# simzero/cudaParticlesFoam

Hardware: AMD Instinct MI355X
Metric: Mparticle-steps/s (higher is better)
Workload: dtype f64

## Files before the change

### cudaparticlesfoam_amd/csrc/cpf_api.cpp

```cpp
#include <hip/hip_runtime.h>

#include <algorithm>
#include <cmath>
#include <cstring>
#include <limits>
#include <condition_variable>
#include <mutex>
#include <string>
#include <thread>
#include <utility>
#include <vector>

#include "cpf.h"
#include "cpf_device.h"
#include "cpf_internal.h"
#include "cpf_own.h"
#include "cpf_philox.h"
#include "cpf_walk.h"

#ifndef CPF_TIMING_EVENT_FLAGS
#define CPF_TIMING_EVENT_FLAGS hipEventReleaseToDevice
#endif

namespace {
// ... 1069 lines not shown
    CPF_REQUIRE(ctx, value != 1 && value != 2 && value != 5, CPF_ERR_ARG,
                "step_variant 1, 2 and 5 are experiments (measured slower on every mesh) and not in this build: make EXPERIMENTS=1");
#endif
    ctx->stepVariant = (int)value;
    return CPF_OK;
}

struct Option {
    const char* key;
    double lo, hi, step;
    const char* message;
    int (*set)(cpf_context*, double);
};
#define CPF_OPT(lvalue, expr) [](cpf_context* c, double v) -> int { c->lvalue = (expr); return CPF_OK; }
constexpr double kTiny = std::numeric_limits<double>::denorm_min(), kHuge = std::numeric_limits<double>::max();
const Option kOptions[] = {
    {"step_variant", -1, 5, 1, "step_variant must be -1..5", setStepVariant},
    {"vertex_fast", 0, 1, 1, "vertex_fast must be 0 or 1", CPF_OPT(vertexFast, v != 0)},
    {"z_fold", 0, 1, 1, "z_fold must be 0 or 1", CPF_OPT(zFold, v != 0)},
    {"mixed_records", 0, 1, 1, "mixed_records must be 0 or 1", CPF_OPT(mixedRecords, v != 0)},
    {"flat_walk", 0, 1, 1, "flat_walk must be 0 or 1", CPF_OPT(streamState.flat, (int)v)},
    {"flat_z", 0, 1, 1, "flat_z must be 0 or 1", CPF_OPT(streamState.flatZ, (int)v)},
    {"box_records", 0, 1, 1, "box_records must be 0 or 1", CPF_OPT(boxRecords, v != 0)},
    {"stream_tiles_per_chunk", 1, 1024, 1, "stream_tiles_per_chunk must be 1..1024", CPF_OPT(streamState.tilesPerChunk, (int)v)},
    {"sort_key_bits", 0, 0, 0, nullptr, setSortKeyBits},
    {"stream_tail_fraction", 0, 1, 0, "stream_tail_fraction must be in [0, 1]", CPF_OPT(streamState.tailFraction, v)},
    {"coop_max_cells", 0, 1 << 24, 0, "coop_max_cells must be in [0, 2^24]", CPF_OPT(streamState.coopMaxCells, (int)v)},
    {"stream_lookup", cpf::kLookupLoop - 1, cpf::kLookupBox, 1, "stream_lookup must be -1 (auto) or 0 ... 6", CPF_OPT(streamState.lookup, (int)v)},
    {"stream_lookup_by_density", 0, 1, 1, "stream_lookup_by_density must be 0 or 1", CPF_OPT(streamState.densityLookup, (int)v)},
    {"sort_method", 0, 2, 2, "sort_method must be 2 (this library's radix sort) or 0 (hipcub's)", CPF_OPT(sortMethod, (int)v)},
    {"sort_curve", -1, 1, 1, "sort_curve must be -1 (by regime), 0 (cell id) or 1 (Morton rank)", CPF_OPT(sortCurve, (int)v)},
    {"vtu_binary", 0, 1, 1, "vtu_binary must be 0 or 1", CPF_OPT(vtuBinary, v != 0)},
    {"stream_debug", 0, 0, 0, nullptr, CPF_OPT(streamState.debug, (int)v)},
    {"stream_waves_per_cu", 0, 32, 1, "stream_waves_per_cu must be 0..32 (0 = auto)", CPF_OPT(streamState.wavesPerCU, (int)v)},
    {"sort_interval", 0, 1e9, 0, "sort_interval must be >= 0 (0 = never)", CPF_OPT(sortInterval, (int)v)},
    {"timing_stride", 1, 1e6, 1, "timing_stride must be an integer >= 1", CPF_OPT(timing.stride, (int)v)},
    {"stats", 0, 0, 0, nullptr, CPF_OPT(stats, v != 0)},
    {"nonplanar_tol", kTiny, kHuge, 0, "nonplanar_tol must be a positive number", CPF_OPT(nonplanarTol, v)},
    {"split_nonplanar", 0, 1, 1, "split_nonplanar must be 0 or 1", CPF_OPT(splitNonplanar, v != 0)},
};
#undef CPF_OPT
}
extern "C" {

int cpf_set_option(cpf_context* ctx, const char* key, double value) {
    CPF_REQUIRE(ctx, ctx && key, CPF_ERR_ARG, "null argument");
    for (const Option& o : kOptions) {
        if (std::strcmp(key, o.key) != 0) continue;
        CPF_REQUIRE(ctx, !o.message || (value >= o.lo && value <= o.hi && (o.step == 0 || std::fmod(value - o.lo, o.step) == 0)),
                    CPF_ERR_ARG, o.message);
        return o.set(ctx, value);
    }
    return fail(ctx, CPF_ERR_ARG, std::string("cpf_set_option: unknown key '") + key + "'");
}

}
namespace cpf {
void set_context_error(cpf_context* ctx, const char* message) {
    if (ctx) ctx->err = message ? message : "";
}
}
extern "C" {

int cpf_step_kernel_name(cpf_context* ctx, double D, unsigned flags, char* buf, size_t bufBytes) {
    CPF_REQUIRE(ctx, ctx && buf && bufBytes > 0, CPF_ERR_ARG, "null argument");
    CPF_REQUIRE(ctx, ctx->mesh.have, CPF_ERR_STATE, "cpf_step_kernel_name: call cpf_set_mesh first");
// ... 664 lines not shown
```

### cudaparticlesfoam_amd/csrc/cpf_device.h

```cpp
#pragma once
#include <hip/hip_runtime.h>

#include <cstdint>
#include <type_traits>
#include <utility>

#include "cpf.h"
#include "cpf_internal.h"

namespace cpf {

constexpr int kBlock = 256;
constexpr int kCounterSlots = 1024;

struct MeshView {
    const int32_t* cellOff;
    const double4* planes;
    const int32_t* nbr;
    const int32_t* groupOff;
    const int32_t* groupNbr;
    const double4* U;
    const double4* cellRec;
    const double4* boxRec;
    int32_t nCells;
    int32_t allHex;
    int32_t zPairLast;
    int32_t zSide0;
    int32_t zThin;
    int32_t mixed;
};

struct GridView {
    double origin[3], invBin[3], lo[3], hi[3];
    int32_t dims[3];
    const int32_t* binOff;
    const int32_t* binCells;
};

constexpr size_t kStreamGrabBytes = 2 * 256 * 16 * sizeof(unsigned);
constexpr int kStreamHitSpillDoubles = 3 * 64;
struct StreamState {
    unsigned* d_grab = nullptr;
    double* d_hitSpill = nullptr;
    int hitSpillWaves = 0;
    int parity = 0;
    int numCU = 256;
    int tilesPerChunk = 0;
    int wavesPerCU = 0;
    int coopMaxCells = 0;
    int lookup = -1;
    double tailFraction = -1.0;
    int debug = 0;
    const volatile unsigned long long* occupiedHost = nullptr;
    int densityLookup = 0;
    bool flatField = false;
    int flat = 1;
    int flatZ = 1;
    unsigned* zBad = nullptr;
};

constexpr int kCoopMaxCells = 1 << 24;
constexpr int kFusedCoopCycles = 1 << 30;
struct VertexField;

enum : int { kLookupLoop = 0, kLookupFixed = 1, kLookupMixedBig = 2, kLookupMixed = 3, kLookupSparse = 4, kLookupMixedLoop = 5,
             kLookupBox = 6, kLookupFlatLoop = 8, kLookupFlatFixed = 9, kLookupBoxGroups = 11 };
struct LookupMode {
    int id;
    bool fixed;
    bool mixed;
    bool bigCells;
    bool box;
    bool flat;
    int gatherAhead;
};
constexpr LookupMode kLookupModes[] = {
    {kLookupLoop,       false, false, false, false, false, 0},
    {kLookupFixed,      true,  false, false, false, false, 0},
    {kLookupMixedBig,   true,  true,  true,  false, false, 0},
    {kLookupMixed,      true,  true,  false, false, false, 0},
    {kLookupSparse,     true,  false, false, false, false, 3},
    {kLookupMixedLoop,  false, true,  false, false, false, 0},
    {kLookupBox,        true,  false, false, true,  false, 0},
    {kLookupFlatLoop,   false, false, false, false, true,  0},
    {kLookupFlatFixed,  true,  false, false, false, true,  0},
// ... 143 lines not shown
```

### cudaparticlesfoam_amd/csrc/cpf_stream.hip

```cpp
#include "cpf_stream_ops.h"

#include <hip/hip_ext.h>

#include <type_traits>

namespace cpf {

#ifndef CPF_STREAM_SLOTS
#define CPF_STREAM_SLOTS 6
#endif
#ifndef CPF_STREAM_SLOTS_FIXED
#define CPF_STREAM_SLOTS_FIXED 9
#endif
#ifndef CPF_STREAM_WAVES
#define CPF_STREAM_WAVES 7
#endif
constexpr int kSlotStride = 8;
#ifndef CPF_STREAM_GATHER_LANES
#define CPF_STREAM_GATHER_LANES 32
#endif
constexpr int kStreamGatherLanes = CPF_STREAM_GATHER_LANES;
#ifndef CPF_STREAM_PAIRED
#define CPF_STREAM_PAIRED 0
#endif
// ... 62 lines not shown
#endif
#ifndef CPF_STREAM_WAVES_L2
#define CPF_STREAM_WAVES_L2 6
#endif
#ifndef CPF_STREAM_WAVES_B0
#define CPF_STREAM_WAVES_B0 7
#endif
#ifndef CPF_STREAM_HIT_POOL_B0
#define CPF_STREAM_HIT_POOL_B0 18
#endif
#ifndef CPF_STREAM_WAVES_FLAT
#define CPF_STREAM_WAVES_FLAT CPF_STREAM_WAVES
#endif
#ifndef CPF_STREAM_WAVES_FLAT_BODY
#define CPF_STREAM_WAVES_FLAT_BODY 0
#endif
#ifndef CPF_FLAT_ROUND_GATHER
#define CPF_FLAT_ROUND_GATHER 1
#endif
#ifndef CPF_FLAT_ROUND_HINTS
#define CPF_FLAT_ROUND_HINTS 1
#endif
#ifndef CPF_FLAT_ROUND_ONE_HOOK
#define CPF_FLAT_ROUND_ONE_HOOK 1
#endif
#ifndef CPF_FLAT_ROUND_MASK
#define CPF_FLAT_ROUND_MASK 1
#endif
#ifndef CPF_FLAT_ROUND_OUTCOME
#define CPF_FLAT_ROUND_OUTCOME 1
#endif
#ifndef CPF_FLAT_FACE_ASM
#define CPF_FLAT_FACE_ASM 1
#endif
#ifndef CPF_STREAM_SLOTS_BROWN
#define CPF_STREAM_SLOTS_BROWN 10
#endif
#ifndef CPF_STREAM_HIT_REGS_L2
#define CPF_STREAM_HIT_REGS_L2 0
#endif
#ifndef CPF_STREAM_WAVES_VERTEX
#define CPF_STREAM_WAVES_VERTEX 4
#endif
template <bool BROWNIAN, bool STORE_VEL, bool STATS, int LOOKUP>
struct StreamShape {
    static constexpr LookupMode mode = lookup_traits(LOOKUP);
    static_assert(mode.id == LOOKUP, "LOOKUP: a mode of kLookupModes");
    static constexpr int slots = [] {
        if (!mode.fixed) return CPF_STREAM_SLOTS;
        if (mode.box) return BROWNIAN ? CPF_STREAM_SLOTS_BOX_B : CPF_STREAM_SLOTS_BOX;
        if (BROWNIAN && LOOKUP == kLookupFixed) return CPF_STREAM_SLOTS_BROWN;
        return CPF_STREAM_SLOTS_FIXED;
    }();
    static_assert(slots >= 4 && slots <= 32, "slots");
    static constexpr int stride = mode.box ? 4 : kSlotStride;
    static constexpr bool hitInRegs = !BROWNIAN && (!mode.bigCells || CPF_STREAM_HIT_REGS_L2);
    static constexpr int pool = [] {
        if (hitInRegs) return 1;
        if (mode.mixed) return 16;
        if (BROWNIAN && LOOKUP == kLookupLoop) return CPF_STREAM_HIT_POOL_B0;
        return CPF_STREAM_HIT_POOL;
    }();
    static constexpr int waves = [] {
        if (STORE_VEL || STATS) return 1;
        if (mode.gatherAhead != 0) return BROWNIAN ? 4 : 5;
        if (BROWNIAN && mode.mixed) return 5;
// ... 19 lines not shown
              shape_is<9>(9, 7, 1, 9, 7, 40) && shape_is<11>(9, 6, 1, 12, 5, 16), "StreamShape: slots, waves, pool per mode");
#endif

template <bool BROWNIAN, bool REFLECT, bool STORE_VEL, bool STATS, int LOOKUP, bool VERTEX, bool ZSET = false>
__device__ __forceinline__ void stream_body(
    const int64_t* __restrict__ gid, double* __restrict__ vel, int64_t n, double dt, double sigma, uint32_t step0,
    int nCyc, uint32_t seed, const MeshView& m, unsigned long long* __restrict__ counters, const StreamArgs& sa, const VertexField& vf) {
    using Shape = StreamShape<BROWNIAN, STORE_VEL, STATS, LOOKUP>;
    constexpr bool LOOKUP_FIXED = Shape::mode.fixed, mixed = Shape::mode.mixed, bigCells = Shape::mode.bigCells, BOX = Shape::mode.box;
    constexpr bool FLAT = Shape::mode.flat, HIT_IN_REGS = Shape::hitInRegs;
    constexpr int kGatherAhead = Shape::mode.gatherAhead, NS = Shape::slots, kStride = Shape::stride, kPool = Shape::pool;
    constexpr unsigned kRecBytes = 32u * kStride;
    constexpr unsigned ALL = NS == 32 ? 0xFFFFFFFFu : ((1u << NS) - 1u);
    __shared__ double4 slots[NS][kStride];
    __shared__ unsigned sCnt[4];
    constexpr bool kInRound = CPF_STREAM_INROUND == 2 || (CPF_STREAM_INROUND == 1 && BROWNIAN);
    static_assert(!(kInRound && mixed), "in-round reflection knows neither face groups nor two-record cells");
    static_assert(!ZSET || (FLAT && !BROWNIAN && !VERTEX), "settled z: the flat walk without the kick or the vertex advect");
    __shared__ double sLane[ZSET ? 2 : 3][64];
    __shared__ double sPool[3][kPool];
    __shared__ unsigned sPoolUsed;
    __shared__ double sPre[ZSET ? 160 : (BROWNIAN ? 288 : 224)];
    __shared__ double sCone[VERTEX ? kVertexBlocks : 1][VERTEX ? kVertexTets * 10 : 1];
    double(*sE)[64] = sLane;
    const int lane = threadIdx.x;
    const unsigned ul = threadIdx.x;
    const unsigned preBase = uniform32(lds_addr(sPre));
    const unsigned slotBase = uniform32(lds_addr(slots));
    const int tpc = sa.tilesPerChunk;
    constexpr bool kMaskBusy = ZSET && CPF_FLAT_ROUND_MASK != 0, kPlainOutcome = ZSET && CPF_FLAT_ROUND_OUTCOME != 0;
    constexpr bool kFlatGather = ZSET && CPF_FLAT_ROUND_GATHER != 0, kHints = ZSET && CPF_FLAT_ROUND_HINTS != 0;
    constexpr bool kOneHook = ZSET && CPF_FLAT_ROUND_ONE_HOOK != 0;
    constexpr bool kFaceAsm = ZSET && CPF_FLAT_FACE_ASM != 0 && CPF_STREAM_FLAT_ZERO_SKIP == 0;
    const bool zKeep = ZSET || (FLAT && CPF_STREAM_FLAT_Z != 0 && sa.zSettled != 0);
    auto park = [&](const D3& e) __attribute__((always_inline)) {
        sE[0][lane] = e.x; sE[1][lane] = e.y;
        if (!ZSET) sE[2][lane] = e.z;
    };
    auto parked = [&]() __attribute__((always_inline)) -> D3 {
        if (ZSET) return {sE[0][lane], sE[1][lane], 0.0};
        return {sE[0][lane], sE[1][lane], sE[2][lane]};
    };
    const bool zFold = !BOX && BROWNIAN && REFLECT && m.zThin != 0;
    const bool zLast = !FLAT && !BROWNIAN && m.zPairLast != 0;
    const bool flatKick = zFold && m.zSide0 != 0;
    const unsigned nTiles = (unsigned)((n + 63) >> 6);
    const unsigned nFull = (unsigned)(n >> 6), nTail = (unsigned)n & 63u;
    const unsigned big = sa.bigChunks;
    const unsigned nChunks = big + (nTiles - big * (unsigned)tpc);
    auto chunk_first = [&](unsigned c) -> unsigned {
        return c < big ? c * (unsigned)tpc : big * (unsigned)tpc + (c - big);
    };
    auto chunk_tiles = [&](unsigned c, unsigned firstTile) -> int {
        if (c >= nChunks) return 0;
        const unsigned k = nTiles - firstTile;
        const unsigned want = c < big ? (unsigned)tpc : 1u;
        return (int)(k < want ? k : want);
    };
    auto chunk_of = [&](unsigned j) -> unsigned {
        const unsigned long long c = (unsigned long long)(blockIdx.x & (kStreamGroups - 1)) + (unsigned long long)kStreamGroups * j;
        return c < (unsigned long long)nChunks ? (unsigned)c : nChunks;
    };
    StepStats st = {0, 0, 0, 0};
#ifdef CPF_STREAM_TIMELINE
    const uint64_t tl0 = __builtin_amdgcn_s_memrealtime();
    unsigned tlTiles = 0, tlRounds = 0;
    unsigned tlWaitRec = 0, tlWaitEnd = 0, tlMissRounds = 0;
    unsigned long long* const tlH = (!STORE_VEL && vel != nullptr && (sa.debug & 4)) ? reinterpret_cast<unsigned long long*>(vel) + 8 * 16384 : nullptr;
    unsigned tlVis = 0, tlRoundIdx = 0;
#endif

    for (unsigned k = blockIdx.x; k < (unsigned)kStreamGroups; k += gridDim.x)
        if (lane == 0) sa.grabNext[k * kStreamCounterStride] = 0u;
    const unsigned grp = blockIdx.x & (kStreamGroups - 1);
    unsigned* const myGrab = sa.grab + grp * kStreamCounterStride;

    auto prefetch = [&](unsigned t, const CloudPtrs& cp) __attribute__((always_inline)) -> int {
        double* const x = cp.x; double* const y = cp.y; double* const z = cp.z; int32_t* const cell = cp.cell;
        t = uniform32(t);
        const int64_t b = (int64_t)t * 64;
        unsigned ul = threadIdx.x;
        asm volatile("" : "+v"(ul));
        if (t < nFull) {
            const char* s1 = (ul < 32u ? reinterpret_cast<const char*>(x + b) : reinterpret_cast<const char*>(y + b)) + (ul & 31u) * 16u;
            glds16(s1, preBase);
            if (zKeep) {
                if (ul < 16u) glds16(reinterpret_cast<const char*>(cell + b) + ul * 16u, preBase + 1024u);
            } else if (ul < 48u) {
                const char* s2 = ul < 32u ? reinterpret_cast<const char*>(z + b) + ul * 16u
                                          : reinterpret_cast<const char*>(cell + b) + (ul - 32u) * 16u;
                glds16(s2, preBase + 1024u);
            }
            if (BROWNIAN) {
                const int64_t* const g = CPF_STREAM_BROWN_KERNARG ? static_cast<const int64_t*>(kernarg_pointer<kKernArgGid>()) : gid;
                if (g != nullptr) {
                    if (ul < 32u) glds16(reinterpret_cast<const char*>(g + b) + ul * 16u, preBase + 1792u);
                    return 3;
                }
            }
            return 2;
        }
        const unsigned lim = nTail - 1u;
        const unsigned l = ul < lim ? ul : lim;
        if (zKeep) {
            const double vx = (x + b)[l], vy = (y + b)[l];
            const int vc = (cell + b)[l];
            sPre[ul] = vx; sPre[64 + ul] = vy;
            reinterpret_cast<int*>(sPre + 128)[ul] = vc;
        } else {
        const double vx = (x + b)[l], vy = (y + b)[l], vz = (z + b)[l];
        const int vc = (cell + b)[l];
        sPre[ul] = vx; sPre[64 + ul] = vy; sPre[128 + ul] = vz;
        reinterpret_cast<int*>(sPre + 192)[ul] = vc;
        }
        if (BROWNIAN) {
            const int64_t* const g = CPF_STREAM_BROWN_KERNARG ? static_cast<const int64_t*>(kernarg_pointer<kKernArgGid>()) : gid;
            if (g != nullptr) reinterpret_cast<int64_t*>(sPre + 224)[ul] = (g + b)[l];
        }
        return 0;
    };
// ... 29 lines not shown
                const bool haveIds = (CPF_STREAM_BROWN_KERNARG ? kernarg_pointer<kKernArgGid>() : (void*)gid) != nullptr;
                pid = haveIds ? (uint64_t) reinterpret_cast<const int64_t*>(sPre + 224)[ul] : (uint64_t)tile * 64 + ul;
            }
            if (ul > plim || pc < 0) pc = CPF_CELL_FROZEN;
            if (FLAT && !ZSET && !zKeep && ballot64(pc >= 0 && !(fabs(pz) <= 1.7976931348623157e308)) != 0ull) {
                unsigned* const bad = static_cast<unsigned*>(kernarg_pointer<kKernArgZBad>());
                if (bad != nullptr && lane == 0) *bad = 1u;
            }

            int cur = pc;
            int key2 = 0, carNext = 0, carBest = -1;
            double carDT = 2.0;
            D3 S_ = {px, py, pz}, v = {0, 0, 0};
            const uint64_t id = pid;

            unsigned ntile = 0;
            int ntilesLeft = 0;

            auto hook = [&](const D3& prev) __attribute__((always_inline)) -> int {
                int younger = 0;
                __builtin_amdgcn_sched_barrier(0);
                if (tilesLeft > 1) {
                    ntile = tile + 1;
                    ntilesLeft = tilesLeft - 1;
                } else {
                    unsigned got = 0;
                    if (lane == 0) got = grab_sync(myGrab);
                    const unsigned nxt = chunk_of(uniform32(got));
                    ntile = chunk_first(nxt);
                    ntilesLeft = chunk_tiles(nxt, ntile);
                }
                const CloudPtrs cp = kernarg_cloud_ptrs();
                double* const x = cp.x; double* const y = cp.y; double* const z = cp.z; int32_t* const cell = cp.cell;
                if (havePrev && !(sa.debug & 1)) {
                    const int64_t b = (int64_t)uniform32(rtile) * 64;
                    if (STORE_VEL && ralive) {
                        double* vv = vel + 3 * b;
                        async_store(vv, ul * 24u, rvx); async_store(vv + 1, ul * 24u, rvy); async_store(vv + 2, ul * 24u, rvz);
                    }
                    if (ul <= rlim) {
                        async_store(x + b, ul * 8u, prev.x); async_store(y + b, ul * 8u, prev.y);
                        if (!zKeep) async_store(z + b, ul * 8u, prev.z);
                        async_store(cell + b, ul * 4u, rc);
                    }
                    younger += zKeep ? 3 : 4;
                }
                if (ntilesLeft > 0 && !(sa.debug & 2)) younger += prefetch(ntile, cp);
                __builtin_amdgcn_sched_barrier(0);
                return younger;
            };

            bool busy = false;
            unsigned long long busyM = 0ull;
            bool zUnclear = false;
            int token = INT32_MIN, h = 0, j = 0;
            int hitAt = -1;
            D3 hitReg = {0, 0, 0};
            auto park_hit = [&](const D3& Hp) __attribute__((always_inline)) {
                if (HIT_IN_REGS) { hitReg = Hp; return; }
                if (hitAt < 0) hitAt = (int)atomicAdd(&sPoolUsed, 1u);
                if (hitAt < kPool) { sPool[0][hitAt] = Hp.x; sPool[1][hitAt] = Hp.y; sPool[2][hitAt] = Hp.z; }
                else {
                    double* sp = static_cast<double*>(kernarg_pointer<kKernArgHitSpill>()) + (size_t)blockIdx.x * kStreamHitSpillDoubles;
                    async_store(sp, ul * 8u, Hp.x); async_store(sp + 64, ul * 8u, Hp.y); async_store(sp + 128, ul * 8u, Hp.z);
                }
            };
// ... 109 lines not shown
                        }
#endif
                    }
                } else {
                    unsigned long long todo = busyMask;
                    missLanes = 0ull;
                    while (todo != 0ull) {
                        const int leader = __ffsll((long long)todo) - 1;
                        const int ck = __builtin_amdgcn_readlane(lk, leader);
                        const bool mine = lk == ck;
                        const unsigned long long same = ballot64(mine) & busyMask;
                        const unsigned long long hitTag = __builtin_amdgcn_uicmp((unsigned)tagv, (unsigned)ck, 32 );
                        if (hitTag != 0ull) {
                            const int sl = __ffsll((long long)hitTag) - 1;
                            used |= 1u << sl;
                            if (mine) myslot = sl;
                        } else {
                            missLanes |= same;
                        }
                        todo &= ~same;
                    }
                }
                int nJobs = 0;
                if (missLanes != 0ull) {
#define CPF_JOB(J)                                                                                          \
                    if (missLanes != 0ull && used != ALL) {                                                 \
                        const int leader = __ffsll((long long)missLanes) - 1;                               \
                        const int ck = __builtin_amdgcn_readlane(lk, leader);                               \
                        const unsigned cand = ~used & ALL;                                                  \
                        const unsigned hi = cand & (ALL << fifo) & ALL;                                     \
                        const int victim = __ffs((int)(hi ? hi : cand)) - 1;                                \
                        fifo = (unsigned)(victim + 1) == (unsigned)NS ? 0u : (unsigned)(victim + 1);          \
                        used |= 1u << victim;                                                               \
                        if (lane == victim) tagv = ck;                                                      \
                        const bool mine = lk == ck;                                                         \
                        if (mine) myslot = victim;                                                          \
                        missLanes &= ~ballot64(mine);                                                       \
                        if (ul < kRecBytes / 16u)                                                            \
                            glds16(reinterpret_cast<const char*>(BOX ? m.boxRec : m.cellRec) + (int64_t)ck * kRecBytes + ul * 16u,  \
                                   uniform32(slotBase + (unsigned)victim * kRecBytes));                     \
                        nJobs = J + 1;                                                                      \
                    }
                    CPF_JOB(0) CPF_JOB(1) CPF_JOB(2) CPF_JOB(3)
                    if (LOOKUP_FIXED) { CPF_JOB(4) CPF_JOB(5) CPF_JOB(6) CPF_JOB(7) }
#undef CPF_JOB
                }
                int younger = 0;
                if (hookDue) younger = hook(Epre);
                if (BROWNIAN && cycleStart && busy) {
                    uint32_t kStep0 = step0, kSeed = seed;
                    if (CPF_STREAM_BROWN_KERNARG) kernarg_u32_pair<kKernArgStep0, kKernArgSeed>(kStep0, kSeed);
                    const D3 xi = normal3(id, kStep0 + (uint32_t)c, kSeed);
                    sE[0][lane] = xi.x; sE[1][lane] = xi.y; sE[2][lane] = xi.z;
                }
#ifdef CPF_STREAM_TIMELINE
                const uint64_t tlw0 = __builtin_amdgcn_s_memrealtime();
#endif
                if (nJobs != 0) {
                    if (ZSET) {
                        if (younger == 5) wait_vmcnt<5>();
                        else if (younger == 3) wait_vmcnt<3>();
                        else if (younger == 2) wait_vmcnt<2>();
                        else wait_vmcnt<0>();
                    } else
                    if (younger >= 7) wait_vmcnt<7>();
                    else if (younger == 6) wait_vmcnt<6>();
                    else if (younger == 5) wait_vmcnt<5>();
                    else if (younger >= 4) wait_vmcnt<4>();
                    else if (younger == 3) wait_vmcnt<3>();
                    else if (younger >= 2) wait_vmcnt<2>();
                    else wait_vmcnt<0>();
#ifdef CPF_STREAM_TIMELINE
                    tlWaitRec += (unsigned)(__builtin_amdgcn_s_memrealtime() - tlw0); ++tlMissRounds;
#endif
                }
                const bool gatherRound = __popcll(missLanes) >= kStreamGatherLanes;
                auto advect = [&](const double4* rec) __attribute__((always_inline)) -> D3 {
                    D3 Pn;
                    if (VERTEX) {
                        Pn = {S_.x + dt * v.x, S_.y + dt * v.y, S_.z + dt * v.z};
                    } else {
                        double4 u;
                        if (BOX) { const double2 uxy = reinterpret_cast<const double2*>(rec)[5]; u = {uxy.x, uxy.y, reinterpret_cast<const double*>(rec)[12], 0.0}; }
                        else u = rec[6];
                        v = {u.x, u.y, u.z};
                        if (ZSET) Pn = {fma(dt, v.x, S_.x), fma(dt, v.y, S_.y), 0.0};
                        else Pn = axpy(dt, v, S_);
                    }
                    D3 disp = {Pn.x - S_.x, Pn.y - S_.y, ZSET ? 0.0 : Pn.z - S_.z};
                    if (BROWNIAN) {
                        const D3 xi = {sE[0][lane], sE[1][lane], sE[2][lane]};
// ... 204 lines not shown
                    }
#endif
                    if (live > 0) cycle_end();
#ifdef CPF_STREAM_CAP_TEST
                    if (capDropped) { S_ = capKeep; cur = capCur; }
#endif
                }
            } else {
                const D3 prev = parked();
                (void)hook(prev);
            }

#ifdef CPF_STREAM_TIMELINE
            const uint64_t tle0 = __builtin_amdgcn_s_memrealtime();
#endif
            wait_vmcnt<0>();
#ifdef CPF_STREAM_TIMELINE
            tlWaitEnd += (unsigned)(__builtin_amdgcn_s_memrealtime() - tle0);
            ++tlTiles;
#endif
            rtile = tile; havePrev = true;
            park(S_);
            if (STORE_VEL) { rvx = v.x; rvy = v.y; rvz = v.z; ralive = pc >= 0; }
            rc = cur;
            rlim = plim;
            if (ntilesLeft <= 0) break;
            tile = ntile; tilesLeft = ntilesLeft;
        }
        {
            const int64_t b = (int64_t)rtile * 64;
            const CloudPtrs cp = kernarg_cloud_ptrs();
            double* const x = cp.x; double* const y = cp.y; double* const z = cp.z; int32_t* const cell = cp.cell;
            const D3 res = parked();
            if (ul <= rlim) {
                (x + b)[ul] = res.x; (y + b)[ul] = res.y;
                if (!zKeep) (z + b)[ul] = res.z;
                (cell + b)[ul] = rc;
            }
            if (STORE_VEL && ralive) {
                double* vv = vel + 3 * b;
                vv[3 * ul] = rvx; vv[3 * ul + 1] = rvy; vv[3 * ul + 2] = rvz;
            }
        }
    }
#ifdef CPF_STREAM_TIMELINE
    if (!STORE_VEL && vel != nullptr && lane == 0) {
        uint64_t* o = reinterpret_cast<uint64_t*>(vel) + 8 * (uint64_t)blockIdx.x;
        o[0] = tl0; o[1] = __builtin_amdgcn_s_memrealtime(); o[2] = tlTiles; o[3] = tlRounds;
        o[4] = tlWaitRec; o[5] = tlWaitEnd; o[6] = tlMissRounds; o[7] = 0;
    }
#endif
    if (STATS) flush_stats(st, counters, sCnt);
}

template <bool BROWNIAN, bool REFLECT, bool STORE_VEL, bool STATS, int LOOKUP>
__global__ __launch_bounds__(64, (StreamShape<BROWNIAN, STORE_VEL, STATS, LOOKUP>::waves)) void step_kernel_stream(
    double* __restrict__ , double* __restrict__ , double* __restrict__ , int32_t* __restrict__ ,
    const int64_t* __restrict__ gid, double* __restrict__ vel, int64_t n, double dt, double sigma, uint32_t step0,
    int nCyc, uint32_t seed, MeshView m, unsigned long long* __restrict__ counters, StreamArgs sa) {
    stream_body<BROWNIAN, REFLECT, STORE_VEL, STATS, LOOKUP, false>(gid, vel, n, dt, sigma, step0, nCyc, seed, m, counters, sa, VertexField{});
}

template <bool BROWNIAN, bool REFLECT, bool STORE_VEL, bool STATS, int LOOKUP>
__global__ __launch_bounds__(64, ((STORE_VEL || STATS) ? 1 : CPF_STREAM_WAVES_VERTEX)) void step_kernel_stream_vertex(
    double* __restrict__ , double* __restrict__ , double* __restrict__ , int32_t* __restrict__ ,
    const int64_t* __restrict__ gid, double* __restrict__ vel, int64_t n, double dt, double sigma, uint32_t step0,
    int nCyc, uint32_t seed, MeshView m, unsigned long long* __restrict__ counters, StreamArgs sa, VertexField vf) {
    stream_body<BROWNIAN, REFLECT, STORE_VEL, STATS, LOOKUP, true>(gid, vel, n, dt, sigma, step0, nCyc, seed, m, counters, sa, vf);
}

template <bool REFLECT, bool STORE_VEL, bool STATS, int LOOKUP>
__global__ __launch_bounds__(64, (StreamShape<false, STORE_VEL, STATS, LOOKUP>::waves)) void step_kernel_stream_flat(
    double* __restrict__ , double* __restrict__ , double* __restrict__ , int32_t* __restrict__ ,
    const int64_t* __restrict__ gid, double* __restrict__ vel, int64_t n, double dt, double sigma, uint32_t step0,
// ... 22 lines not shown
        else if constexpr (ZS) return &step_kernel_stream_flat<R_, SV, ST, LF>;
        else return &step_kernel_stream<B, R_, SV, ST, LF>;
    }();
    static int wavesPerCU = 0;
    if (wavesPerCU == 0) {
        int nb = 0;
        const hipError_t e = hipOccupancyMaxActiveBlocksPerMultiprocessor(&nb, kernel, 64, 0);
        if (e != hipSuccess) return e;
        wavesPerCU = nb < 1 ? 1 : (nb > 32 ? 32 : nb);
        if (ZS && CPF_STREAM_WAVES_FLAT_BODY > 0 && wavesPerCU > 4 * CPF_STREAM_WAVES_FLAT_BODY) wavesPerCU = 4 * CPF_STREAM_WAVES_FLAT_BODY;
    }
    const int64_t nTiles = (n + 63) >> 6;
    if (nTiles >= ((int64_t)1 << 31)) return hipErrorInvalidValue;
    const int64_t slotsOnChip = (int64_t)((ss.wavesPerCU > 0 && !VX) ? ss.wavesPerCU : wavesPerCU) * ss.numCU;
    int tpc = ss.tilesPerChunk > 0 ? ss.tilesPerChunk : (!mode.fixed ? 4 : 3);
    const double tailFraction = ss.tailFraction >= 0.0 ? ss.tailFraction : (!mode.fixed ? 0.1 : 0.2);
    while (tpc > 1 && nTiles / tpc < 4 * slotsOnChip) tpc = tpc > 2 ? tpc - 1 : 1;
    int64_t bigChunks = (int64_t)((double)(nTiles / tpc) * (1.0 - tailFraction));
    if (tpc == 1 || bigChunks < 0) bigChunks = 0;
    const int64_t nChunks = bigChunks + (nTiles - bigChunks * tpc);
    int64_t R = slotsOnChip / kStreamGroups;
    const int64_t need = (nChunks + kStreamGroups - 1) / kStreamGroups;
    if (R > need) R = need;
    if (R < 1) R = 1;
    unsigned* cur = ss.d_grab + (size_t)(ss.parity & 1) * kStreamGroups * kStreamCounterStride;
    unsigned* nxt = ss.d_grab + (size_t)((ss.parity & 1) ^ 1) * kStreamGroups * kStreamCounterStride;
    if (R * kStreamGroups > ss.hitSpillWaves) R = ss.hitSpillWaves / kStreamGroups;
    if (R < 1 || ss.d_hitSpill == nullptr) return hipErrorInvalidValue;
    const bool zSettled = mode.flat && !VX && settled && ss.flatZ != 0;
    if (ZS != zSettled && mode.flat && !VX) return hipErrorInvalidValue;
    StreamArgs sa = {cur, nxt, (int)R, tpc, (unsigned)bigChunks, ss.debug, ss.d_hitSpill, zSettled ? 1 : 0, ss.zBad};
    auto launch = [&](const auto&... tail) {
        const dim3 grid((unsigned)(R * kStreamGroups));
        if (evStart != nullptr && evStop != nullptr)
            hipExtLaunchKernelGGL(kernel, grid, dim3(64), 0, st, evStart, evStop, 0, x, y, z, cell, gid, vel, n, dt, sigma, step0, nCyc,
                                  seed, m, counters, sa, tail...);
        else
            hipLaunchKernelGGL(kernel, grid, dim3(64), 0, st, x, y, z, cell, gid, vel, n, dt, sigma, step0, nCyc, seed, m, counters, sa,
                               tail...);
        return stream_launch_done(st, ss);
    };
    if constexpr (VX) return vf == nullptr ? hipErrorInvalidValue : launch(*vf);
    else return launch();
}

static int stream_lookup_mode(int64_t n, const MeshView& m, const StreamState& ss, bool brown, bool vertex) {
    int64_t cells = m.nCells;
    if (ss.densityLookup && ss.occupiedHost != nullptr) {
        const int64_t occ = (int64_t)ss.occupiedHost[0], live = (int64_t)ss.occupiedHost[1];
        if (occ > 0 && occ <= cells && live > 0 && live <= 2 * n && n <= 2 * live) cells = occ;
    }
    if (vertex) {
        if (ss.lookup == kLookupLoop || ss.lookup == kLookupFixed) return ss.lookup;
        return n < 128 * cells ? kLookupFixed : kLookupLoop;
    }
    if (m.mixed == 1 && m.boxRec != nullptr && m.zThin == 0 && ss.lookup < 0) return kLookupBoxGroups;
    if (m.mixed == 2) return kLookupMixedBig;
    if (m.mixed) return (ss.lookup >= 0 ? ss.lookup == kLookupLoop : n >= 128 * cells) ? kLookupMixedLoop : kLookupMixed;
    const bool box = m.boxRec != nullptr && m.zThin == 0;
    if (ss.lookup >= 0) return (ss.lookup == kLookupBox && !box) ? kLookupFixed : ss.lookup;
    if (box && CPF_STREAM_BOX_SPARSE) return kLookupBox;
    if (n < kStreamSparsePerCell * cells) return kLookupSparse;
    const bool flat = !brown && ss.flat && ss.flatField && m.zSide0 != 0;
    if (n < 128 * cells) return flat ? kLookupFlatFixed : kLookupFixed;
    return flat ? kLookupFlatLoop : kLookupLoop;
}

StepPlan plan_step(const MeshView& m, const StreamState& ss, int variant, const VertexField* vf, int64_t n, int nCyc, double D,
                   unsigned flags, bool stats) {
    StepPlan p;
    p.brown = D > 0.0;
    p.reflect = (flags & CPF_STEP_NO_REFLECT) == 0;
    p.storeVel = (flags & CPF_STEP_STORE_VEL) != 0;
    p.stats = stats;
    const int coopMaxCells = (ss.coopMaxCells <= 0 || ss.coopMaxCells > kCoopMaxCells) ? kCoopMaxCells : ss.coopMaxCells;
    if (!m.allHex) {
// ... 11 lines not shown
    if (vf != nullptr) {
        p.cone = vf->cone != nullptr;
        const bool streams = p.cone && vf->tetsPerCell == 12 && m.mixed == 0 && m.cellRec != nullptr && variant == kVariantStream;
        p.kernel = streams ? StepPlan::kStreamVertex : StepPlan::kVertex;
        if (streams) p.lookup = stream_lookup_mode(n, m, ss, p.brown, true);
        return p;
    }
    if (variant == kVariantAhead && (p.brown || p.storeVel || nCyc != 1)) variant = kVariantStream;
    p.kernel = (StepPlan::Kernel)variant;
    if (variant == kVariantStream) p.lookup = stream_lookup_mode(n, m, ss, p.brown, false);
    return p;
}

constexpr bool vertex_mode(LookupMode r) { return !(r.mixed || r.box || r.flat || r.gatherAhead != 0); }
hipError_t launch_step_stream(const StepPlan& p, hipStream_t st, double* x, double* y, double* z, int32_t* cell, const int64_t* gid,
                              double* vel, int64_t n, double dt, double sigma, uint32_t step0, int nCyc, uint32_t seed,
                              const MeshView& m, unsigned long long* counters, const VertexField* vf, StreamState& ss, bool zSettled,
                              hipEvent_t evStart, hipEvent_t evStop) {
    return with_bools([&](auto B, auto R, auto SV, auto ST) {
        auto inst = [&](auto kick, auto LF, auto VX, auto ZS) {
            return launch_stream_inst<kick, R, SV, ST, LF, VX, ZS>(st, x, y, z, cell, gid, vel, n, dt, sigma, step0, nCyc, seed, m, counters,
                                                                   ss, vf, zSettled, evStart, evStop);
        };
        constexpr std::true_type yes{}; constexpr std::false_type no{};
        if (p.kernel == StepPlan::kStreamVertex)
            return with_lookup(p.lookup, [&](auto LF) {
                if constexpr (vertex_mode(lookup_traits(LF))) return inst(B, LF, yes, no);
                else return hipErrorInvalidValue;
            });
        const bool body = p.flat_body(ss, zSettled);
        return with_lookup(p.lookup, [&](auto LF) {
            if constexpr (!lookup_traits(LF).flat) return inst(B, LF, no, no);
            else if constexpr (B) return hipErrorInvalidValue;
            else return body ? inst(no, LF, no, yes) : inst(no, LF, no, no);
        });
    }, p.brown, p.reflect, p.storeVel, p.stats);
}

}
```

### cudaparticlesfoam_amd/csrc/cpf_stream_ops.h

```cpp
#pragma once
#include "cpf_walk.h"

namespace cpf {

#ifndef CPF_STREAM_GROUPS
#define CPF_STREAM_GROUPS 256
#endif
constexpr int kStreamGroups = CPF_STREAM_GROUPS;
constexpr int kStreamCounterStride = 16;

typedef __attribute__((address_space(3))) const char* lds_cptr;
__device__ __forceinline__ unsigned lds_addr(const void* p) {
    return (unsigned)(uintptr_t)(lds_cptr)p;
}
__device__ __forceinline__ unsigned uniform32(unsigned v) { return (unsigned)__builtin_amdgcn_readfirstlane((int)v); }
__device__ __forceinline__ int64_t uniform64(int64_t v) {
    const unsigned lo = uniform32((unsigned)v), hi = uniform32((unsigned)((uint64_t)v >> 32));
    return (int64_t)(((uint64_t)hi << 32) | lo);
}
__device__ __forceinline__ void glds16(const void* gsrc, unsigned ldsDst) {
    unsigned keep;
    asm volatile("s_waitcnt lgkmcnt(0)\n\ts_mov_b32 %0, m0\n\ts_mov_b32 m0, %2\n\ts_nop 0\n\t"
                 "global_load_lds_dwordx4 %1, off\n\ts_mov_b32 m0, %0"
                 : "=&s"(keep) : "v"(gsrc), "s"(ldsDst) : "memory");
}
__device__ __forceinline__ void async_store(double* base, unsigned byteOff, double v) {
    asm volatile("s_nop 4\n\tglobal_store_dwordx2 %0, %1, %2" : : "v"(byteOff), "v"(v), "s"(base) : "memory");
}
__device__ __forceinline__ void async_store(int32_t* base, unsigned byteOff, int v) {
    asm volatile("s_nop 4\n\tglobal_store_dword %0, %1, %2" : : "v"(byteOff), "v"(v), "s"(base) : "memory");
}
__device__ __forceinline__ unsigned grab_sync(unsigned* base) {
    unsigned r;
    asm volatile("s_nop 4\n\tglobal_atomic_add %0, %1, %2, %3 sc0\n\ts_waitcnt vmcnt(0)" : "=&v"(r) : "v"(0u), "v"(1u), "s"(base) : "memory");
    return r;
}
__device__ __forceinline__ void load3_sync(const double* base, unsigned byteOff, double& a, double& b, double& c) {
    asm volatile("s_waitcnt vmcnt(0)\n\ts_nop 4\n\tglobal_load_dwordx2 %0, %3, %4 sc0 sc1\n\tglobal_load_dwordx2 %1, %3, %4 offset:512 sc0 sc1\n\t"
                 "global_load_dwordx2 %2, %3, %4 offset:1024 sc0 sc1\n\ts_waitcnt vmcnt(0)"
                 : "=&v"(a), "=&v"(b), "=&v"(c) : "v"(byteOff), "s"(base) : "memory");
}
struct CloudPtrs { double* x; double* y; double* z; int32_t* cell; };
__device__ __forceinline__ CloudPtrs kernarg_cloud_ptrs() {
    typedef unsigned u32x8 __attribute__((ext_vector_type(8)));
    u32x8 r;
    asm volatile("s_load_dwordx8 %0, %1, 0x0\n\ts_waitcnt lgkmcnt(0)" : "=s"(r) : "s"(__builtin_amdgcn_kernarg_segment_ptr()) : "memory");
    auto ptr = [](unsigned lo, unsigned hi) { return (uintptr_t)(((unsigned long long)hi << 32) | lo); };
    return {reinterpret_cast<double*>(ptr(r[0], r[1])), reinterpret_cast<double*>(ptr(r[2], r[3])),
            reinterpret_cast<double*>(ptr(r[4], r[5])), reinterpret_cast<int32_t*>(ptr(r[6], r[7]))};
}
template <int BYTE_OFFSET>
__device__ __forceinline__ void* kernarg_pointer() {
    typedef unsigned u32x2 __attribute__((ext_vector_type(2)));
    u32x2 r;
    asm volatile("s_load_dwordx2 %0, %1, %2\n\ts_waitcnt lgkmcnt(0)" : "=s"(r) : "s"(__builtin_amdgcn_kernarg_segment_ptr()), "n"(BYTE_OFFSET) : "memory");
    return reinterpret_cast<void*>((uintptr_t)(((unsigned long long)r[1] << 32) | r[0]));
}
template <int OFF_A, int OFF_B>
__device__ __forceinline__ void kernarg_u32_pair(uint32_t& a, uint32_t& b) {
    asm volatile("s_load_dword %0, %2, %3\n\ts_load_dword %1, %2, %4\n\ts_waitcnt lgkmcnt(0)"
                 : "=&s"(a), "=&s"(b) : "s"(__builtin_amdgcn_kernarg_segment_ptr()), "n"(OFF_A), "n"(OFF_B) : "memory");
}
template <int BYTE_OFFSET>
__device__ __forceinline__ double kernarg_f64() {
    typedef unsigned u32x2 __attribute__((ext_vector_type(2)));
    u32x2 r;
    asm volatile("s_load_dwordx2 %0, %1, %2\n\ts_waitcnt lgkmcnt(0)" : "=s"(r) : "s"(__builtin_amdgcn_kernarg_segment_ptr()), "n"(BYTE_OFFSET) : "memory");
    return __longlong_as_double((long long)(((unsigned long long)r[1] << 32) | r[0]));
}
template <int N>
__device__ __forceinline__ void wait_vmcnt() { asm volatile("s_waitcnt vmcnt(%0)" : : "n"(N) : "memory"); }

struct StreamArgs {
    unsigned* grab;
    unsigned* grabNext;
    int wavesPerGroup;
    int tilesPerChunk;
    unsigned bigChunks;
    int debug;
    double* hitSpill;
    int zSettled;
    unsigned* zBad;
};

inline hipError_t stream_launch_done(hipStream_t st, StreamState& ss) {
    const hipError_t e = hipGetLastError();
    if (e == hipSuccess) { ss.parity ^= 1; return e; }
    (void)hipMemsetAsync(ss.d_grab, 0, kStreamGrabBytes, st);
    return e;
}

}
```

Measured before the change: 112,400.

## Use 32-bit offsets in flat settled-z stream walk, segmenting large clouds

Adds a 32-bit offset path for the flat settled-z stream kernel. Tile loads, stores and record gathers compute unsigned byte offsets instead of 64-bit pointer arithmetic, and stores are fused into inline-asm groups. The m0-based global_load_lds variant and a branchy scalar vmcnt wait are meant to trim scalar and address instructions in the hot loop. To keep offsets within 32 bits, clouds larger than a segment size (new option) are launched in several kernels, which adds launches and splits the event timing across first and last launches.

After: 112,900 (median of 6 runs). Within noise of the previous version (+0.5%).

```diff
diff --git a/cudaparticlesfoam_amd/csrc/cpf_api.cpp b/cudaparticlesfoam_amd/csrc/cpf_api.cpp
--- a/cudaparticlesfoam_amd/csrc/cpf_api.cpp
+++ b/cudaparticlesfoam_amd/csrc/cpf_api.cpp
@@ -1125,6 +1125,8 @@
     {"sort_curve", -1, 1, 1, "sort_curve must be -1 (by regime), 0 (cell id) or 1 (Morton rank)", CPF_OPT(sortCurve, (int)v)},
     {"vtu_binary", 0, 1, 1, "vtu_binary must be 0 or 1", CPF_OPT(vtuBinary, v != 0)},
     {"stream_debug", 0, 0, 0, nullptr, CPF_OPT(streamState.debug, (int)v)},
+    {"stream_segment_particles", 64, (double)((int64_t)1 << 29), 0, "stream_segment_particles must be in [64, 2^29]",
+     CPF_OPT(streamState.segment, (int64_t)v / 64 * 64)},
     {"stream_waves_per_cu", 0, 32, 1, "stream_waves_per_cu must be 0..32 (0 = auto)", CPF_OPT(streamState.wavesPerCU, (int)v)},
     {"sort_interval", 0, 1e9, 0, "sort_interval must be >= 0 (0 = never)", CPF_OPT(sortInterval, (int)v)},
     {"timing_stride", 1, 1e6, 1, "timing_stride must be an integer >= 1", CPF_OPT(timing.stride, (int)v)},
diff --git a/cudaparticlesfoam_amd/csrc/cpf_device.h b/cudaparticlesfoam_amd/csrc/cpf_device.h
--- a/cudaparticlesfoam_amd/csrc/cpf_device.h
+++ b/cudaparticlesfoam_amd/csrc/cpf_device.h
@@ -51,6 +51,7 @@
     int lookup = -1;
     double tailFraction = -1.0;
     int debug = 0;
+    int64_t segment = (int64_t)1 << 29;
     const volatile unsigned long long* occupiedHost = nullptr;
     int densityLookup = 0;
     bool flatField = false;
diff --git a/cudaparticlesfoam_amd/csrc/cpf_stream.hip b/cudaparticlesfoam_amd/csrc/cpf_stream.hip
--- a/cudaparticlesfoam_amd/csrc/cpf_stream.hip
+++ b/cudaparticlesfoam_amd/csrc/cpf_stream.hip
@@ -118,6 +118,15 @@
 #endif
 #ifndef CPF_FLAT_FACE_ASM
 #define CPF_FLAT_FACE_ASM 1
+#endif
+#ifndef CPF_FLAT_OFF32
+#define CPF_FLAT_OFF32 1
+#endif
+#ifndef CPF_FLAT_WAIT
+#define CPF_FLAT_WAIT 1
+#endif
+#ifndef CPF_FLAT_GLDS
+#define CPF_FLAT_GLDS 1
 #endif
 #ifndef CPF_STREAM_SLOTS_BROWN
 #define CPF_STREAM_SLOTS_BROWN 10
@@ -203,6 +212,8 @@
     constexpr bool kFlatGather = ZSET && CPF_FLAT_ROUND_GATHER != 0, kHints = ZSET && CPF_FLAT_ROUND_HINTS != 0;
     constexpr bool kOneHook = ZSET && CPF_FLAT_ROUND_ONE_HOOK != 0;
     constexpr bool kFaceAsm = ZSET && CPF_FLAT_FACE_ASM != 0 && CPF_STREAM_FLAT_ZERO_SKIP == 0;
+    constexpr bool kOff32 = ZSET && CPF_FLAT_OFF32 != 0;
+    constexpr bool kLeanWait = ZSET && CPF_FLAT_WAIT != 0, kGldsM0 = ZSET && CPF_FLAT_GLDS != 0;
     const bool zKeep = ZSET || (FLAT && CPF_STREAM_FLAT_Z != 0 && sa.zSettled != 0);
     auto park = [&](const D3& e) __attribute__((always_inline)) {
         sE[0][lane] = e.x; sE[1][lane] = e.y;
@@ -229,6 +240,11 @@
         return (int)(k < want ? k : want);
     };
     auto chunk_of = [&](unsigned j) -> unsigned {
+        if (kOff32) {
+            constexpr unsigned jMax = 0xFFFFFFFFu / (unsigned)kStreamGroups;
+            const unsigned c = (blockIdx.x & (kStreamGroups - 1)) | ((j < jMax ? j : jMax) * (unsigned)kStreamGroups);
+            return c < nChunks ? c : nChunks;
+        }
         const unsigned long long c = (unsigned long long)(blockIdx.x & (kStreamGroups - 1)) + (unsigned long long)kStreamGroups * j;
         return c < (unsigned long long)nChunks ? (unsigned)c : nChunks;
     };
@@ -252,11 +268,27 @@
         const int64_t b = (int64_t)t * 64;
         unsigned ul = threadIdx.x;
         asm volatile("" : "+v"(ul));
+        if (kOff32) {
+            const unsigned o8 = t * 512u, o4 = t * 256u;
+            if (t < nFull) {
+                glds16_as<kGldsM0>((ul < 32u ? reinterpret_cast<const char*>(x) : reinterpret_cast<const char*>(y)) + (o8 + (ul & 31u) * 16u), preBase);
+                if (ul < 16u) glds16_as<kGldsM0>(reinterpret_cast<const char*>(cell) + (o4 + ul * 16u), preBase + 1024u);
+                return 2;
+            }
+            const unsigned lim = nTail - 1u;
+            const unsigned l = ul < lim ? ul : lim;
+            const double vx = *reinterpret_cast<const double*>(reinterpret_cast<const char*>(x) + (o8 + l * 8u));
+            const double vy = *reinterpret_cast<const double*>(reinterpret_cast<const char*>(y) + (o8 + l * 8u));
+            const int vc = *reinterpret_cast<const int*>(reinterpret_cast<const char*>(cell) + (o4 + l * 4u));
+            sPre[ul] = vx; sPre[64 + ul] = vy;
+            reinterpret_cast<int*>(sPre + 128)[ul] = vc;
+            return 0;
+        }
         if (t < nFull) {
             const char* s1 = (ul < 32u ? reinterpret_cast<const char*>(x + b) : reinterpret_cast<const char*>(y + b)) + (ul & 31u) * 16u;
-            glds16(s1, preBase);
+            glds16_as<kGldsM0>(s1, preBase);
             if (zKeep) {
-                if (ul < 16u) glds16(reinterpret_cast<const char*>(cell + b) + ul * 16u, preBase + 1024u);
+                if (ul < 16u) glds16_as<kGldsM0>(reinterpret_cast<const char*>(cell + b) + ul * 16u, preBase + 1024u);
             } else if (ul < 48u) {
                 const char* s2 = ul < 32u ? reinterpret_cast<const char*>(z + b) + ul * 16u
                                           : reinterpret_cast<const char*>(cell + b) + (ul - 32u) * 16u;
@@ -352,6 +384,12 @@
                 }
                 const CloudPtrs cp = kernarg_cloud_ptrs();
                 double* const x = cp.x; double* const y = cp.y; double* const z = cp.z; int32_t* const cell = cp.cell;
+                if (kOff32 && havePrev && !(sa.debug & 1)) {
+                    const unsigned rt = uniform32(rtile);
+                    if (STORE_VEL && ralive) async_store3_at(vel, rt * 1536u + ul * 24u, rvx, rvy, rvz);
+                    if (ul <= rlim) async_store3(x, y, cell, rt * 512u + ul * 8u, rt * 256u + ul * 4u, prev.x, prev.y, rc);
+                    younger += 3;
+                } else
                 if (havePrev && !(sa.debug & 1)) {
                     const int64_t b = (int64_t)uniform32(rtile) * 64;
                     if (STORE_VEL && ralive) {
@@ -527,13 +565,16 @@
                         const int victim = __ffs((int)(hi ? hi : cand)) - 1;                                \
                         fifo = (unsigned)(victim + 1) == (unsigned)NS ? 0u : (unsigned)(victim + 1);          \
                         used |= 1u << victim;                                                               \
-                        if (lane == victim) tagv = ck;                                                      \
+                        unsigned ckv = (unsigned)ck;               \
+                        if (kOff32) asm("" : "+v"(ckv));           \
+                        if (lane == victim) tagv = (int)ckv;                                                \
                         const bool mine = lk == ck;                                                         \
                         if (mine) myslot = victim;                                                          \
                         missLanes &= ~ballot64(mine);                                                       \
                         if (ul < kRecBytes / 16u)                                                            \
-                            glds16(reinterpret_cast<const char*>(BOX ? m.boxRec : m.cellRec) + (int64_t)ck * kRecBytes + ul * 16u,  \
-                                   uniform32(slotBase + (unsigned)victim * kRecBytes));                     \
+                            glds16_as<kGldsM0>(reinterpret_cast<const char*>(BOX ? m.boxRec : m.cellRec) +                \
+                                     (kOff32 ? (int64_t)((uint64_t)ckv * kRecBytes) : (int64_t)ck * kRecBytes) + ul * 16u,    \
+                                 uniform32(slotBase + (unsigned)victim * kRecBytes));                       \
                         nJobs = J + 1;                                                                      \
                     }
                     CPF_JOB(0) CPF_JOB(1) CPF_JOB(2) CPF_JOB(3)
@@ -552,6 +593,7 @@
                 const uint64_t tlw0 = __builtin_amdgcn_s_memrealtime();
 #endif
                 if (nJobs != 0) {
+                    if (kLeanWait) wait_vmcnt_0_2_5(younger); else
                     if (ZSET) {
                         if (younger == 5) wait_vmcnt<5>();
                         else if (younger == 3) wait_vmcnt<3>();
@@ -822,6 +864,18 @@
             const CloudPtrs cp = kernarg_cloud_ptrs();
             double* const x = cp.x; double* const y = cp.y; double* const z = cp.z; int32_t* const cell = cp.cell;
             const D3 res = parked();
+            if (kOff32) {
+                const unsigned o8 = rtile * 512u + ul * 8u;
+                if (ul <= rlim) {
+                    *reinterpret_cast<double*>(reinterpret_cast<char*>(x) + o8) = res.x;
+                    *reinterpret_cast<double*>(reinterpret_cast<char*>(y) + o8) = res.y;
+                    *reinterpret_cast<int*>(reinterpret_cast<char*>(cell) + (o8 >> 1)) = rc;
+                }
+                if (STORE_VEL && ralive) {
+                    double* vv = reinterpret_cast<double*>(reinterpret_cast<char*>(vel) + (rtile * 1536u + ul * 24u));
+                    vv[0] = rvx; vv[1] = rvy; vv[2] = rvz;
+                }
+            } else {
             if (ul <= rlim) {
                 (x + b)[ul] = res.x; (y + b)[ul] = res.y;
                 if (!zKeep) (z + b)[ul] = res.z;
@@ -830,6 +884,7 @@
             if (STORE_VEL && ralive) {
                 double* vv = vel + 3 * b;
                 vv[3 * ul] = rvx; vv[3 * ul + 1] = rvy; vv[3 * ul + 2] = rvz;
+            }
             }
         }
     }
@@ -918,7 +973,7 @@
     StreamArgs sa = {cur, nxt, (int)R, tpc, (unsigned)bigChunks, ss.debug, ss.d_hitSpill, zSettled ? 1 : 0, ss.zBad};
     auto launch = [&](const auto&... tail) {
         const dim3 grid((unsigned)(R * kStreamGroups));
-        if (evStart != nullptr && evStop != nullptr)
+        if (evStart != nullptr || evStop != nullptr)
             hipExtLaunchKernelGGL(kernel, grid, dim3(64), 0, st, evStart, evStop, 0, x, y, z, cell, gid, vel, n, dt, sigma, step0, nCyc,
                                   seed, m, counters, sa, tail...);
         else
@@ -928,6 +983,26 @@
     };
     if constexpr (VX) return vf == nullptr ? hipErrorInvalidValue : launch(*vf);
     else return launch();
+}
+
+constexpr int64_t kFlatSegmentMax = (int64_t)1 << 29, kFlatSegmentMaxVel = (int64_t)1 << 27;
+template <bool R_, bool SV, bool ST, int LF>
+static hipError_t launch_stream_flat(hipStream_t st, double* x, double* y, double* z, int32_t* cell, const int64_t* gid, double* vel,
+                                     int64_t n, double dt, double sigma, uint32_t step0, int nCyc, uint32_t seed, const MeshView& m,
+                                     unsigned long long* counters, StreamState& ss, bool settled, hipEvent_t evStart, hipEvent_t evStop) {
+    const int64_t most = SV ? kFlatSegmentMaxVel : kFlatSegmentMax;
+    const int64_t seg = (ss.segment < 64 ? 64 : (ss.segment > most ? most : ss.segment)) & ~(int64_t)63;
+    if (CPF_FLAT_OFF32 == 0 || n <= seg)
+        return launch_stream_inst<false, R_, SV, ST, LF, false, true>(st, x, y, z, cell, gid, vel, n, dt, sigma, step0, nCyc, seed, m, counters,
+                                                                      ss, nullptr, settled, evStart, evStop);
+    for (int64_t at = 0; at < n; at += seg) {
+        const int64_t k = n - at < seg ? n - at : seg;
+        const hipError_t e = launch_stream_inst<false, R_, SV, ST, LF, false, true>(
+            st, x + at, y + at, z + at, cell + at, gid != nullptr ? gid + at : nullptr, vel != nullptr ? vel + 3 * at : nullptr, k, dt, sigma,
+            step0, nCyc, seed, m, counters, ss, nullptr, settled, at == 0 ? evStart : nullptr, at + k >= n ? evStop : nullptr);
+        if (e != hipSuccess) return e;
+    }
+    return hipSuccess;
 }
 
 static int stream_lookup_mode(int64_t n, const MeshView& m, const StreamState& ss, bool brown, bool vertex) {
@@ -1005,7 +1080,9 @@
         return with_lookup(p.lookup, [&](auto LF) {
             if constexpr (!lookup_traits(LF).flat) return inst(B, LF, no, no);
             else if constexpr (B) return hipErrorInvalidValue;
-            else return body ? inst(no, LF, no, yes) : inst(no, LF, no, no);
+            else if (body) return launch_stream_flat<R, SV, ST, LF>(st, x, y, z, cell, gid, vel, n, dt, sigma, step0, nCyc, seed, m, counters, ss,
+                                                                    zSettled, evStart, evStop);
+            else return inst(no, LF, no, no);
         });
     }, p.brown, p.reflect, p.storeVel, p.stats);
 }
diff --git a/cudaparticlesfoam_amd/csrc/cpf_stream_ops.h b/cudaparticlesfoam_amd/csrc/cpf_stream_ops.h
--- a/cudaparticlesfoam_amd/csrc/cpf_stream_ops.h
+++ b/cudaparticlesfoam_amd/csrc/cpf_stream_ops.h
@@ -24,11 +24,26 @@
                  "global_load_lds_dwordx4 %1, off\n\ts_mov_b32 m0, %0"
                  : "=&s"(keep) : "v"(gsrc), "s"(ldsDst) : "memory");
 }
+__device__ __forceinline__ void glds16_m0(const void* gsrc, unsigned ldsDst) {
+    asm volatile("s_waitcnt lgkmcnt(0)\n\ts_nop 0\n\tglobal_load_lds_dwordx4 %0, off" : : "v"(gsrc), "{m0}"(ldsDst) : "memory");
+}
+template <bool IN_M0>
+__device__ __forceinline__ void glds16_as(const void* gsrc, unsigned ldsDst) {
+    if constexpr (IN_M0) glds16_m0(gsrc, ldsDst); else glds16(gsrc, ldsDst);
+}
 __device__ __forceinline__ void async_store(double* base, unsigned byteOff, double v) {
     asm volatile("s_nop 4\n\tglobal_store_dwordx2 %0, %1, %2" : : "v"(byteOff), "v"(v), "s"(base) : "memory");
 }
 __device__ __forceinline__ void async_store(int32_t* base, unsigned byteOff, int v) {
     asm volatile("s_nop 4\n\tglobal_store_dword %0, %1, %2" : : "v"(byteOff), "v"(v), "s"(base) : "memory");
+}
+__device__ __forceinline__ void async_store3(double* x, double* y, int32_t* cell, unsigned off8, unsigned off4, double vx, double vy, int c) {
+    asm volatile("global_store_dwordx2 %0, %2, %5\n\tglobal_store_dwordx2 %0, %3, %6\n\tglobal_store_dword %1, %4, %7"
+                 : : "v"(off8), "v"(off4), "v"(vx), "v"(vy), "v"(c), "s"(x), "s"(y), "s"(cell) : "memory");
+}
+__device__ __forceinline__ void async_store3_at(double* base, unsigned byteOff, double a, double b, double c) {
+    asm volatile("global_store_dwordx2 %0, %1, %4\n\tglobal_store_dwordx2 %0, %2, %4 offset:8\n\tglobal_store_dwordx2 %0, %3, %4 offset:16"
+                 : : "v"(byteOff), "v"(a), "v"(b), "v"(c), "s"(base) : "memory");
 }
 __device__ __forceinline__ unsigned grab_sync(unsigned* base) {
     unsigned r;
@@ -71,6 +86,13 @@
 template <int N>
 __device__ __forceinline__ void wait_vmcnt() { asm volatile("s_waitcnt vmcnt(%0)" : : "n"(N) : "memory"); }
 
+__device__ __forceinline__ void wait_vmcnt_0_2_5(int younger) {
+    asm volatile("s_cmp_lt_i32 %0, 5\n\ts_cbranch_scc1 .Lcpf_wait_a%=\n\ts_waitcnt vmcnt(5)\n\ts_branch .Lcpf_wait_z%=\n"
+                 ".Lcpf_wait_a%=:\n\ts_cmp_lt_i32 %0, 2\n\ts_cbranch_scc1 .Lcpf_wait_b%=\n\ts_waitcnt vmcnt(2)\n\ts_branch .Lcpf_wait_z%=\n"
+                 ".Lcpf_wait_b%=:\n\ts_waitcnt vmcnt(0)\n.Lcpf_wait_z%=:"
+                 : : "s"(younger) : "scc", "memory");
+}
+
 struct StreamArgs {
     unsigned* grab;
     unsigned* grabNext;
```
